# sk4161/EgoScaler

Hardware: AMD Instinct MI355X
Metric: clips/sec/GPU (8-frame 224^2, 16-token text) fwd+bwd (higher is better)
Workload: dtype bf16

## Files before the change

### egoscaler_amd/csrc/elementwise.hip

```cpp
#include "common.h"
#include <math.h>

template <typename T>
__global__ __launch_bounds__(256) void layernorm_fwd_kernel(const T* x, const T* add, const T* w, const T* b, T* sum_out, T* y,
                                                            int rows, int cols, float eps) {
    const int row = blockIdx.x * 4 + (threadIdx.x >> 6), lane = threadIdx.x & 63;
    if (row >= rows) return;
    const T* xr = x + (long long)row * cols;
    const T* ar = add ? add + (long long)row * cols : nullptr;
    float s = 0.f;
    for (int c = lane; c < cols; c += 64) {
        float v = Cvt<T>::ld(xr + c);
        if (ar) v += Cvt<T>::ld(ar + c);
        s += v;
    }
    const float mean = wave_sum(s) / cols;
    float q = 0.f;
    for (int c = lane; c < cols; c += 64) {
        float v = Cvt<T>::ld(xr + c);
        if (ar) v += Cvt<T>::ld(ar + c);
        if (sizeof(T) == 2) v = bf2f(f2bf(v));
        const float dlt = v - mean;
        q += dlt * dlt;
    }
// ... 861 lines not shown
#pragma unroll
        for (int j = 0; j < 4; ++j) {
            float pi = p4[j], mi = m4[j], vi = v4[j];
            adamw_elem(pi, mi, vi, g4[j], lr, b1, b2, eps, wd, bc1, bc2_sqrt, gscale);
            p4[j] = pi; m4[j] = mi; v4[j] = vi;
        }
        reinterpret_cast<f32x4*>(p)[i] = p4; reinterpret_cast<f32x4*>(m)[i] = m4; reinterpret_cast<f32x4*>(v)[i] = v4;
        if (p_model) {
            T o[4];
#pragma unroll
            for (int j = 0; j < 4; ++j) Cvt<T>::st(o + j, p4[j]);
            typedef T tx4 __attribute__((ext_vector_type(4)));
            reinterpret_cast<tx4*>(p_model)[i] = tx4{o[0], o[1], o[2], o[3]};
        }
    }
}

template <typename G>
static int adamw_launch(float* master, void* model_copy, const G* grad, float* m, float* v, int64_t n, float lr, float beta1, float beta2, float eps,
                        float weight_decay, int step, float grad_scale, int copy_dtype, hipStream_t stream) {
    if (!master || !grad || !m || !v) return EGOMI_E_BADARG;
    if (n <= 0 || step <= 0) return EGOMI_E_SHAPE;
    if (model_copy && copy_dtype != EGOMI_F32 && copy_dtype != EGOMI_BF16) return EGOMI_E_BADARG;
    const float bc1 = 1.0f - powf(beta1, (float)step), bc2s = sqrtf(1.0f - powf(beta2, (float)step));
    const long long n4 = n / 4, rest = n - 4 * n4;
    const bool vec = n4 > 0 && (((uintptr_t)master | (uintptr_t)m | (uintptr_t)v) & 15) == 0 && ((uintptr_t)grad & (4 * sizeof(G) - 1)) == 0 &&
                     (!model_copy || (copy_dtype == EGOMI_BF16 && ((uintptr_t)model_copy & 7) == 0));
    if (vec) {
        EGOMI_LAUNCH((adamw_vec4_kernel<bf16_t, G>), dim3(ew_grid(n4)), dim3(256), 0, stream, master, (bf16_t*)model_copy, grad, m, v,
                           n4, lr, beta1, beta2, eps, weight_decay, bc1, bc2s, grad_scale);
        if (rest == 0) return egomi_launch_status();
        master += 4 * n4; grad += 4 * n4; m += 4 * n4; v += 4 * n4; n = rest;
        if (model_copy) model_copy = (bf16_t*)model_copy + 4 * n4;
    }
    if (!model_copy || copy_dtype == EGOMI_F32)
        EGOMI_LAUNCH((adamw_kernel<float, G>), dim3(ew_grid(n)), dim3(256), 0, stream, master, (float*)model_copy, grad, m, v,
                           (long long)n, lr, beta1, beta2, eps, weight_decay, bc1, bc2s, grad_scale);
    else
        EGOMI_LAUNCH((adamw_kernel<bf16_t, G>), dim3(ew_grid(n)), dim3(256), 0, stream, master, (bf16_t*)model_copy, grad, m, v,
                           (long long)n, lr, beta1, beta2, eps, weight_decay, bc1, bc2s, grad_scale);
    return egomi_launch_status();
}

extern "C" int egomi_adamw(float* master, void* model_copy, const float* grad, float* m, float* v, int64_t n, float lr, float beta1,
                           float beta2, float eps, float weight_decay, int step, float grad_scale, int copy_dtype, egomi_stream_t stream) {
    return adamw_launch<float>(master, model_copy, grad, m, v, n, lr, beta1, beta2, eps, weight_decay, step, grad_scale, copy_dtype, (hipStream_t)stream);
}
extern "C" int egomi_adamw_g16(float* master, void* model_copy, const void* grad_bf16, float* m, float* v, int64_t n, float lr, float beta1,
                               float beta2, float eps, float weight_decay, int step, float grad_scale, int copy_dtype, egomi_stream_t stream) {
    return adamw_launch<bf16_t>(master, model_copy, (const bf16_t*)grad_bf16, m, v, n, lr, beta1, beta2, eps, weight_decay, step, grad_scale, copy_dtype,
                                (hipStream_t)stream);
}

template <typename T>
__global__ __launch_bounds__(256) void transpose_kernel(const T* in, int R, int C, long long ldi, T* out, long long ldo) {
    __shared__ T tile[32][33];
    const int c0 = blockIdx.x * 32, r0 = blockIdx.y * 32;
    const int tx = threadIdx.x & 31, ty = threadIdx.x >> 5;
    for (int i = ty; i < 32; i += 8) {
        const int r = r0 + i, c = c0 + tx;
        tile[i][tx] = (r < R && c < C) ? in[(long long)r * ldi + c] : (T)0;
    }
    __syncthreads();
    for (int i = ty; i < 32; i += 8) {
        const int c = c0 + i, r = r0 + tx;
        if (c < C && r < ldo) out[(long long)c * ldo + r] = tile[tx][i];
    }
}

__global__ __launch_bounds__(256) void transpose_bf16_vec_kernel(const bf16_t* in, int R, int C, long long ldi, bf16_t* out, long long ldo) {
    __shared__ __attribute__((aligned(16))) bf16_t tile[64][72];
    const int c0 = blockIdx.x * 64, r0 = blockIdx.y * 64;
    const int t = threadIdx.x;
#pragma unroll
    for (int i = 0; i < 2; ++i) {
        const int r = (t >> 3) + 32 * i, cc = (t & 7) * 8;
        u32x4 v = {0u, 0u, 0u, 0u};
        if (r0 + r < R && c0 + cc < C) v = *reinterpret_cast<const u32x4*>(in + (long long)(r0 + r) * ldi + c0 + cc);
        *reinterpret_cast<u32x4*>(&tile[r][cc]) = v;
    }
    __syncthreads();
#pragma unroll
    for (int i = 0; i < 2; ++i) {
        const int oc = (t >> 3) + 32 * i, rc = (t & 7) * 8;
        if (c0 + oc >= C || r0 + rc >= ldo) continue;
        u32x4 v;
#pragma unroll
        for (int j = 0; j < 4; ++j) v[j] = (uint32_t)tile[rc + 2 * j][oc] | ((uint32_t)tile[rc + 2 * j + 1][oc] << 16);
        *reinterpret_cast<u32x4*>(out + (long long)(c0 + oc) * ldo + r0 + rc) = v;
    }
}

extern "C" int egomi_transpose(const void* in, int R, int C, int64_t ldi, void* out, int64_t ldo, int dtype, egomi_stream_t stream) {
    if (!in || !out) return EGOMI_E_BADARG;
    if (R <= 0 || C <= 0 || ldi < C || ldo < R) return EGOMI_E_SHAPE;
    if (dtype == EGOMI_BF16 && C % 8 == 0 && ldi % 8 == 0 && ldo % 8 == 0 && ((uintptr_t)in % 16) == 0 && ((uintptr_t)out % 16) == 0) {
        dim3 g((C + 63) / 64, (unsigned)((ldo + 63) / 64));
        EGOMI_LAUNCH(transpose_bf16_vec_kernel, g, dim3(256), 0, (hipStream_t)stream, (const bf16_t*)in, R, C, (long long)ldi, (bf16_t*)out, (long long)ldo);
        return egomi_launch_status();
    }
    dim3 grid((C + 31) / 32, (unsigned)((ldo + 31) / 32));
    EGOMI_DISPATCH_DTYPE(dtype, EGOMI_LAUNCH(transpose_kernel<T>, grid, dim3(256), 0, (hipStream_t)stream, (const T*)in, R, C, ldi, (T*)out, ldo));
    return egomi_launch_status();
}

template <typename TI, typename TO>
// ... 148 lines not shown
```

### egoscaler_amd/engine.py

```python
import os
import types
from typing import Dict

import torch

from . import lora, ops
from .config import EgoDims


class Workspace:

    def __init__(self, device):
        self.device = device
        self.bufs: Dict[str, torch.Tensor] = {}

    def get(self, name, shape, dtype, zero=False):
        t = self.bufs.get(name)
        shape = tuple(int(s) for s in shape)
        if t is None or t.shape != shape or t.dtype != dtype:
            t = self.bufs[name] = torch.empty(shape, dtype=dtype, device=self.device)
        if zero:
            t.zero_()
        return t

    def bytes(self):
        return sum(t.numel() * t.element_size() for t in self.bufs.values())


class Engine:
    def __init__(self, dims: EgoDims, params: Dict[str, torch.Tensor], device, dtype):
        self.dims, self.w, self.device, self.dtype = dims, params, device, dtype
        self.ws = Workspace(device)
        self.w8 = None
        self.w4 = None
        self.prepared = False
        self.prepare_epoch = 0
        self.lm_wT, self.lm_wT_stale, self.lm_wT_ver = None, True, None
        self.param_ref = {}
        self.grad_fresh = set()
        self._xt_last = {}
        self.main_grad: Dict[str, torch.Tensor] = {}
        self.layer_flat: Dict[int, torch.Tensor] = {}
        self.trainable: Dict[str, bool] = {}
        self.ctx = None
        self.grad_sync = None
        self.pb_drop_override = None
        self.reduced_grad = {}
        self.layer_offs = {}
        self._direct, self._direct_done = None, set()
        self.layer_final_hook = None
        self.param_events = {}
        self.use_fused_attention = True
        self.use_fused_swiglu = os.environ.get("EGOMI_NO_FUSED_SWIGLU", "0") != "1"
        self.use_tail_fuse = os.environ.get("EGOMI_NO_TAIL_FUSE", "0") != "1"
        self.use_tn = os.environ.get("EGOMI_GEMM_TN", "1") != "0"
        self.use_top_rows = os.environ.get("EGOMI_TOP_ROWS", "1") != "0"
        self.top_rows_taken = 0
        self._top_key = None
        self.pb_trainer = None
        self.defer_splice_check = False
        self.pending_splice = None
        self._splice_host = {}
        self.pb_train_mode = False
        self.prepared_bn_stale = False
        self.fold_stale = False
        self.lora = None
        self.lora_version = 0
        self._lora_ws = None

    @staticmethod
    def param_group_of(name):
        if name.startswith("model.layers."):
            return int(name.split(".")[2])
        if name == "model.embed_tokens.weight":
            return "embed"
        if name in ("model.norm.weight", "lm_head.weight"):
            return "post"
        return "pre"

    def wait_params(self, key):
        ev = self.param_events.pop(key, None)
        if ev is not None:
            torch.cuda.current_stream().wait_event(ev)

    def wait_param_updates(self):
        for key in list(self.param_events):
            self.wait_params(key)

    def _notify(self, name):
        if self.grad_sync is not None and name in self.trainable and name in self.main_grad:
            self.grad_sync.ready(name, self.main_grad[name])

    def _notify_layer(self, l):
        one_rank = self.grad_sync is None or getattr(self.grad_sync, "local", False)
        hook = self.layer_final_hook if one_rank else None
        if self.grad_sync is None or l not in self.layer_flat:
            if hook is not None:
                hook(l)
            return
        if self._direct is not None:
            wire, views = self._direct
            for n, v in views.items():
                if n not in self._direct_done:
                    if n in self.grad_fresh:
                        self.main_grad[n].zero_()
                        self.grad_fresh.discard(n)
                    ops.cast(self.main_grad[n].view(-1), wire.dtype, out=v.view(-1))
                self.reduced_grad[n] = v
            self._direct, self._direct_done = None, set()
            self.grad_sync.ready_resident(f"layer{l}", wire)
            if hook is not None:
                hook(l)
            return
        self.grad_sync.ready_flat(f"layer{l}", self.layer_flat[l])
        if hook is not None:
            hook(l)
    def _begin_direct(self, l):
        self._direct, self._direct_done = None, set()
        gs = self.grad_sync
        if gs is None or not getattr(gs, "resident", False) or not self.use_tn or self.dtype != torch.bfloat16:
            return
        names = [n for n in self.layer_param_names(l) if n in self.trainable]
        if not names:
            return
        if l not in self.layer_flat:
            self._alloc_layer_grads(l)
        if any(self.w[n].dim() == 2 and n not in self.grad_fresh for n in names):
            return
        wire = gs.resident_wire(f"layer{l}", self.layer_flat[l].numel(), self.device)
        if wire is None:
            return
# ... 78 lines not shown
            if t.data_ptr() != end or t.untyped_storage().data_ptr() != t0.untyped_storage().data_ptr():
                return None
            end += t.numel() * t.element_size()
        return torch.as_strided(t0, (sum(t.shape[0] for t in ts), t0.shape[1]), (t0.shape[1], 1))

    def stack_gate_up(self, gate, up):
        if not self.gu_il:
            return torch.cat([gate, up], 0)
        Fd = gate.shape[0]
        return torch.stack([gate.view(Fd // 32, 32, -1), up.view(Fd // 32, 32, -1)], 1).reshape(2 * Fd, -1).contiguous()

    def after_weights_update(self):
        self.lm_wT_stale = True
        if self.lora is not None and any(lora.is_adapter(n) for n in self.trainable):
            self.lora_version += 1
        if not self.prepared:
            return
        if self.pb_trainable:
            self.fold_stale = True
        for nm, wt in self.wT.items():
            if nm in self.trainable:
                ops.transpose(self.w[nm], out=wt)

    def set_trainable(self, names):
        self.trainable = {n: True for n in names}

    def grad_buffer(self, name):
        g = self.main_grad.get(name)
        if g is None:
            if name.startswith("model.layers."):
                self._alloc_layer_grads(int(name.split(".")[2]))
                return self.main_grad[name]
            g = torch.zeros(self.w[name].shape, dtype=torch.float32, device=self.device)
            self.main_grad[name] = g
        return g

    def _alloc_layer_grads(self, l):
        names = [n for n in self.layer_param_names(l) if n in self.trainable]
        offs, total = [], 0
        for n in names:
            offs.append(total)
            total += (self.w[n].numel() + 63) // 64 * 64
        flat = torch.zeros(total, dtype=torch.float32, device=self.device)
        self.layer_flat[l] = flat
        self.layer_offs[l] = dict(zip(names, offs))
        for n, o in zip(names, offs):
            self.main_grad[n] = flat[o:o + self.w[n].numel()].view(self.w[n].shape)

    def zero_grad(self):
        self.wait_param_updates()
        for g in self.main_grad.values():
            g.zero_()
        self.grad_fresh.clear()

    def lazy_zero_ok(self, name):
        return self.w[name].dim() == 2 and (name.startswith("model.layers.") or name == "lm_head.weight" or name.startswith("model.point_proj."))

    def flush_fresh(self):
        for n in list(self.grad_fresh):
            self.main_grad[n].zero_()
        self.grad_fresh.clear()

    def _attention(self, qkv, B, S, H, hd, out, causal, key_mask, scale, keep_P):
        d = H * hd
        T = self.dtype
        q, k, v = qkv[:, :d], qkv[:, d:2 * d], qkv[:, 2 * d:]
        sc = self.ws.get("att_scores", (B * H, S, S), torch.float32)
        ops.gemm_raw(q, k, sc, S, S, hd, 3 * d, 3 * d, S, 0, 0, alpha=scale, batch=B * H, batch_inner=H,
                     strides=(S * 3 * d, hd, S * 3 * d, hd, H * S * S, S * S))
        Pm = torch.empty(B * H, S, S, dtype=T, device=self.device) if keep_P else self.ws.get("att_P", (B * H, S, S), T)
        ops.softmax(sc, B * H, H, S, S, Pm, causal=causal, key_mask=key_mask)
        ops.gemm_raw(Pm, v, out, S, hd, S, S, 3 * d, d, 0, 1, batch=B * H, batch_inner=H,
                     strides=(H * S * S, S * S, S * 3 * d, hd, S * d, hd))
        return Pm

    def _attention_bwd(self, qkv, Pm, d_out, dqkv, B, S, H, hd, scale):
        d = H * hd
        q, k, v = qkv[:, :d], qkv[:, d:2 * d], qkv[:, 2 * d:]
        dq, dk, dv = dqkv[:, :d], dqkv[:, d:2 * d], dqkv[:, 2 * d:]
        dP = self.ws.get("att_scores", (B * H, S, S), torch.float32)
        ops.gemm_raw(d_out, v, dP, S, S, hd, d, 3 * d, S, 0, 0, batch=B * H, batch_inner=H,
                     strides=(S * d, hd, S * 3 * d, hd, H * S * S, S * S))
        dS = self.ws.get("att_dS", (B * H, S, S), self.dtype)
        ops.softmax_bwd(Pm, dP, dS, B * H * S, S)
        st_ss = (H * S * S, S * S)
        ops.gemm_raw(dS, k, dq, S, hd, S, S, 3 * d, 3 * d, 0, 1, alpha=scale, batch=B * H, batch_inner=H,
                     strides=(*st_ss, S * 3 * d, hd, S * 3 * d, hd))
        ops.gemm_raw(dS, q, dk, S, hd, S, S, 3 * d, 3 * d, 1, 1, alpha=scale, batch=B * H, batch_inner=H,
                     strides=(*st_ss, S * 3 * d, hd, S * 3 * d, hd))
        ops.gemm_raw(Pm, d_out, dv, S, hd, S, S, d, 3 * d, 1, 1, batch=B * H, batch_inner=H,
                     strides=(*st_ss, S * d, hd, S * 3 * d, hd))

    @torch.no_grad()
    def pointnet(self, nb2d, BG, K):
        if not self.prepared:
            self.prepare()
        if self.fold_stale:
            self.fold_batchnorm()
        w, pb, T, ws, f = self.w, self.dims.pb, self.dtype, self.ws, self.folded
        pre = "model.point_backbone."
        h1 = ops.linear_smallk(nb2d, f["c1_w"], f["c1_b"], act=ops.ACT_RELU, out=ws.get("pn_h1", (BG * K, pb.pn_c1), T))
        h2 = ops.mm(h1, f["c2_w"], out=ws.get("pn_h2", (BG * K, pb.pn_c2), T), bias=w[pre + "encoder.first_conv.3.bias"])
        cat = ops.group_max(h2, BG, K, pb.pn_c2, concat=True, out=ws.get("pn_cat", (BG * K, 2 * pb.pn_c2), T))
        h3 = ops.mm(cat, f["c3_w"], out=ws.get("pn_h3", (BG * K, pb.pn_c3), T), bias=f["c3_b"], act=ops.ACT_RELU)
        h4 = ops.mm(h3, f["c4_w"], out=ws.get("pn_h4", (BG * K, pb.encoder_dims), T), bias=w[pre + "encoder.second_conv.3.bias"])
        return ops.group_max(h4, BG, K, pb.encoder_dims, out=ws.get("pn_tok", (BG, pb.encoder_dims), T))
# ... 480 lines not shown
            else:
                ops.swiglu_bwd(d_act, gu[:, :Fd], gu[:, Fd:], dgu[:, :Fd], dgu[:, Fd:])
        self._wgrad(p + "down_proj.weight", dx, lc["act"])
        names = [p + "gate_proj.weight", p + "up_proj.weight"]
        d_h2, t_h2 = self._stacked_dgrad(dgu, wguT, self.wgu_cat.get(l) if self.prepared else None, names, ws.get("d_h" + sfx, (Ml, d), T),
                                         pl.defer_b and "gu" not in la, **mm)
        if "gu" in la:
            self._lora_bwd(l, "gu", dgu, lc["h2"], d_h2, lT["gu"], il=lc["gu_il"])
        self._wgrad_stacked(names, dgu, lc["h2"])
        n2 = f"model.layers.{l}.post_attention_layernorm.weight"
        return ops.rmsnorm_bwd(d_h2, lc["x_mid"], w[n2], lc["rstd2"], dx_add=dx, dw=self.grad_buffer(n2) if n2 in self.trainable else None,
                               out=ws.get("dx_b" + sfx, (Ml, d), T), tail=t_h2)

    def _attn_half_bwd(self, l, d_mid, lc, pl, key_mask):
        w, lm, T, ws, lw, la = self.w, self.dims.lm, self.dtype, self.ws, pl.layers[l], pl.la
        d, H, hd, B, S, M = lm.hidden_size, lm.num_attention_heads, lm.head_dim, pl.B, pl.S, pl.M
        p, qkv, lT = f"model.layers.{l}.self_attn.", lc["qkv"], lc["lora_T"]
        d_ao = self._dgrad(d_mid, p + "o_proj.weight", ws.get("d_ao" + ("_rows_top" if lw.top else ""), (lw.rows, d), T), **lw.mm)
        if "o" in la:
            self._lora_bwd(l, "o", d_mid, lc["ao"], d_ao, lT["o"])
        self._wgrad(p + "o_proj.weight", d_mid, lc["ao"])
        if lw.top:
            d_ao, d_mid = self._top_window(pl, self._top_buffers(B, S, pl.R)[2:], (d_ao, d_mid), scatter=True)
        dqkv = ws.get("dqkv", (M, 3 * d), T)
        if lc["lse"] is not None:
            ops.attn_bwd(qkv, lc["ao"], lc["lse"], d_ao, dqkv, ws.get("att_delta", (B, H, S), torch.float32), B, S, H, hd, hd ** -0.5,
                         causal=True, key_mask=key_mask, rope=(self.cos, self.sin), q_rows=pl.R if lw.top else 0)
        else:
            self._attention_bwd(qkv, lc["P"], d_ao, dqkv, B, S, H, hd, hd ** -0.5)
            ops.rope_(dqkv, self.cos, self.sin, M, S, 0, 2 * H, hd, 3 * d, inverse=True)
        names = [p + f"{nm}_proj.weight" for nm in "qkv"]
        stack = self.wqkv.get(l) if self.prepared and self.use_tn and T == torch.bfloat16 else None
        d_h, t_h = self._stacked_dgrad(dqkv, self.wqkvT.get(l) if self.prepared else None, stack, names, ws.get("d_h", (M, d), T),
                                       pl.defer_b and "qkv" not in la)
        if "qkv" in la:
            self._lora_bwd(l, "qkv", dqkv, lc["h"], d_h, lT["qkv"])
        self._wgrad_stacked(names, dqkv, lc["h"])
        n1 = f"model.layers.{l}.input_layernorm.weight"
        return ops.rmsnorm_bwd(d_h, lc["x_in"], w[n1], lc["rstd1"], dx_add=d_mid, dw=self.grad_buffer(n1) if n1 in self.trainable else None,
                               out=ws.get("dx_a", (M, d), T), tail=t_h)

    def _layer_bwd(self, l, dx, pl, ctx):
        lc = ctx["layers"][l]
        self._begin_direct(l)
        dx = self._attn_half_bwd(l, self._mlp_bwd(l, dx, lc, pl), lc, pl, ctx["key_mask"])
        self._notify_layer(l)
        return dx

    def _points_bwd(self, dx, ctx):
        w, pb, T, ws, tr = self.w, self.dims.pb, self.dtype, self.ws, self.trainable
        B, S, Bc, Pn, d = ctx["B"], ctx["S"], ctx["n_clouds"], pb.point_token_len, dx.shape[1]
        emb_name = "model.embed_tokens.weight"
        d_feats = ws.get("d_pp_out", (Bc * Pn, d), T, zero=True) if ctx["has_points"] else None
        ops.embed_splice_bwd(dx.view(B, S, d), ctx["ids"], ctx["start_pos"], Pn, self.dims.lm.vocab_size,
                             self.grad_buffer(emb_name) if emb_name in tr else None, d_feats, cloud_idx=ctx["cloud_idx"])
        if d_feats is None:
            return
        acts, g = ctx["pp_acts"], d_feats
        for j in range(len(pb.projection_hidden_dim), -1, -1):
            Wn, bn = f"model.point_proj.{2 * j}.weight", f"model.point_proj.{2 * j}.bias"
            self._wgrad(Wn, g, acts[2 * j])
            self._bgrad(bn, g)
            if j > 0:
                if T == torch.bfloat16:
                    wt = ops.transpose(w[Wn], out=ws.get(f"pp_wT{j}", (w[Wn].shape[1], w[Wn].shape[0]), T))
                    g_in = ops.mm(g, wt, out=ws.get(f"d_pp_act{j}", (Bc * Pn, w[Wn].shape[1]), T))
                else:
                    g_in = ops.mm(g, w[Wn], out=ws.get(f"d_pp_act{j}", (Bc * Pn, w[Wn].shape[1]), T), b_layout=1)
                g = ops.gelu_bwd(g_in, acts[2 * j - 1], out=ws.get(f"d_pp_pre{j}", g_in.shape, T))
            elif ctx.get("pb_ctx") is not None:
                d_backbone = ops.mm(g, w[Wn], b_layout=1)
                self.pb_trainer.backward(d_backbone.view(Bc, Pn, pb.trans_dim), ctx["pb_ctx"])
                if self.grad_sync is not None:
                    for nm in tr:
                        if nm.startswith("model.point_backbone."):
                            self._notify(nm)

    def backward_hidden(self, d_hn):
        ctx, w, ws, pl = self.ctx, self.w, self.ws, self.ctx["plan"]
        nf = "model.norm.weight"
        dx = ops.rmsnorm_bwd(d_hn, ctx["x_last"], w[nf], ctx["rstd_f"], dw=self.grad_buffer(nf) if nf in self.trainable else None,
                             out=ws.get("dx_a" + pl.layers[-1].sfx, ctx["x_last"].shape, self.dtype),
                             window=(pl.S, pl.R) if pl.R else None)
        for l in reversed(range(len(pl.layers))):
            dx = self._layer_bwd(l, dx, pl, ctx)
        self._points_bwd(dx, ctx)
        if self.grad_sync is not None:
            self._notify("model.embed_tokens.weight")
            self._notify(nf)
            for j in range(len(self.dims.pb.projection_hidden_dim) + 1):
                self._notify(f"model.point_proj.{2 * j}.weight")
                self._notify(f"model.point_proj.{2 * j}.bias")
            self.grad_sync.flush()
        self.ctx = None

    def layer_param_names(self, l):
        p = f"model.layers.{l}."
        names = [p + f"self_attn.{n}_proj.weight" for n in "qkvo"] + [p + f"mlp.{n}_proj.weight" for n in ("gate", "up", "down")] + \
                [p + "input_layernorm.weight", p + "post_attention_layernorm.weight"]
        if self.lora is not None:
            names += [n for t in self.lora.targets for n in lora.adapter_names(l, t)]
        return names

    def backward_logits(self, d_logits, hn):
        W = self.w["lm_head.weight"]
        V, d = W.shape
# ... 21 lines not shown
```

### egoscaler_amd/ops.py

```python
import ctypes
import math

import torch

from . import _abi, _lib
from ._lib import c_p, c_i, c_d, c_f, c_sz, c_i64, call, query

F32, BF16 = _abi.EGOMI_F32, _abi.EGOMI_BF16


def dt(t: torch.dtype) -> int:
    if t == torch.float32:
        return F32
    if t == torch.bfloat16:
        return BF16
    raise TypeError(f"unsupported dtype {t}")


def P(t):
    if t is None:
        return c_p(None)
    if not t.is_cuda:
        raise _lib.EgomiError("egoscaler_amd ops need CUDA/HIP tensors (no CPU fallback)")
    return c_p(t.data_ptr())
# ... 433 lines not shown
    call("egomi_gelu_bwd", dy, x, out, x.numel(), dt(x.dtype), S())
    return out


def softmax(scores, Z, heads, Sq, Sk, out, causal=False, q_offset=0, key_mask=None):
    call("egomi_softmax_fwd", scores, Sk, key_mask, Z, heads, Sq, Sk, int(causal), q_offset, out, Sk, dt(out.dtype), S())
    return out


def softmax_bwd(Pm, dP, dS, rows, Sk):
    call("egomi_softmax_bwd", Pm, Sk, dP, Sk, dS, Sk, rows, Sk, dt(Pm.dtype), S())
    return dS


def splice_scan(ids, tok, Pn, n_clouds=None):
    B, Sl = ids.shape
    sp, err, cloud, scratch = (torch.empty(B, dtype=torch.int32, device=ids.device) for _ in range(4))
    call("egomi_splice_scan", ids, B, Sl, tok.point_patch, tok.point_start, tok.point_end, Pn, B if n_clouds is None else n_clouds, sp, err, cloud,
         scratch, S())
    return sp, err, cloud


def embed_splice(ids, W, feats, start_pos, Pn, out=None, cloud_idx=None):
    B, Sl = ids.shape
    V, d = W.shape
    out = torch.empty(B, Sl, d, dtype=W.dtype, device=W.device) if out is None else out
    call("egomi_embed_splice_fwd", ids, W, feats, start_pos, cloud_idx, B, Sl, d, Pn, V, out, dt(W.dtype), S())
    return out


def embed_splice_bwd(dout, ids, start_pos, Pn, V, dW=None, dfeats=None, cloud_idx=None):
    B, Sl, d = dout.shape
    call("egomi_embed_splice_bwd", dout, ids, start_pos, cloud_idx, B, Sl, d, Pn, V, dW, dfeats, dt(dout.dtype), S())


def cross_entropy(logits, targets, ignore_index, dlogits=None, grad_scale=1.0):
    R, V = logits.shape
    cnt = torch.zeros(1, dtype=torch.int32, device=logits.device)
    ls = torch.zeros(1, dtype=torch.float32, device=logits.device)
    rows = torch.empty(R, dtype=torch.float32, device=logits.device)
    call("egomi_ce_count", targets, R, ignore_index, cnt, S())
    call("egomi_ce_fwd_bwd", logits, _ld(logits), targets, R, V, ignore_index, cnt, ls, rows, dlogits, _ld(dlogits) if dlogits is not None else 0,
         grad_scale, dt(logits.dtype), S())
    return ls, cnt


def adamw(master, model_copy, grad, m, v, lr, beta1, beta2, eps, wd, step, grad_scale=1.0):
    if grad.dtype not in (torch.float32, torch.bfloat16) or not grad.is_contiguous() or grad.numel() != master.numel():
        raise _lib.EgomiError("adamw: the gradient must be a contiguous fp32 or bf16 tensor of the parameter's size")
    call("egomi_adamw" if grad.dtype == torch.float32 else "egomi_adamw_g16", master, model_copy, grad, m, v, master.numel(), lr, beta1, beta2, eps,
         wd, step, grad_scale, dt(model_copy.dtype) if model_copy is not None else F32, S())


def transpose(x, ldo=None, out=None):
    R, C = x.shape
    ldo = R if ldo is None else ldo
    out = torch.empty(C, ldo, dtype=x.dtype, device=x.device) if out is None else out
    call("egomi_transpose", x, R, C, _ld(x), out, ldo, dt(x.dtype), S())
    return out


def cast(x, dtype, out=None):
    out = torch.empty(x.shape, dtype=dtype, device=x.device) if out is None else out
    call("egomi_cast", x, dt(x.dtype), out, dt(dtype), x.numel(), S())
    return out


def rank_sum(chunks, out):
    W, c = chunks.shape
    call("egomi_rank_sum", chunks, dt(chunks.dtype), W, c, out, dt(out.dtype), S())
    return out


def add(a, b, out=None):
    out = torch.empty_like(a) if out is None else out
    call("egomi_add", a, b, out, a.numel(), dt(a.dtype), S())
    return out


def colsum_(x, out):
    R, C = x.shape
    call("egomi_colsum", x, R, C, _ld(x), out, dt(x.dtype), S())
    return out


def group_max(x, BG, M, C, concat=False, out=None):
    if out is None:
        out = torch.empty((BG * M, 2 * C) if concat else (BG, C), dtype=x.dtype, device=x.device)
    call("egomi_group_max", x, BG, M, C, out, int(concat), dt(x.dtype), S())
    return out


def linear_smallk(x, w, b, act=0, out=None):
    R, K = x.numel() // x.shape[-1], x.shape[-1]
    N = w.shape[0]
    out = torch.empty(R, N, dtype=w.dtype, device=w.device) if out is None else out
    call("egomi_linear_smallk", x, dt(x.dtype), w, b, out, R, N, K, act, dt(w.dtype), S())
    return out


AttnDesc = _abi.STRUCTS["egomi_attn_desc"]


def _attn_desc(qkv, B, Sq, H, hd, scale, causal, key_mask):
    d = AttnDesc()
    dm = H * hd
# ... 88 lines not shown
```

### egoscaler_amd/optim.py

```python
import torch

from . import ops


class EgoAdamW:
    def __init__(self, model, lr=2e-5, betas=(0.9, 0.999), eps=1e-8, weight_decay=0.01):
        self.model, self.lr, self.betas, self.eps, self.wd = model, lr, betas, eps, weight_decay
        self.t = 0
        self.state = {}
        for n, p in model.named_parameters():
            if p.requires_grad:
                master = p.data if p.dtype == torch.float32 else p.data.float()
                self.state[n] = {"p": p, "master": master, "m": torch.zeros_like(master), "v": torch.zeros_like(master)}

    def arm(self, grad_scale=1.0, lr=None):
        eng = self.model.engine
        self._armed = None
        eng.layer_final_hook = None
        if (eng.grad_sync is not None and not getattr(eng.grad_sync, "local", False)) or eng.device.type != "cuda" or not eng.any_layer_trainable:
            return False
        if any(nm in eng.trainable for nm in getattr(eng, "wT", {})):
            return False
        groups = {}
        for n in self.state:
            groups.setdefault(eng.param_group_of(n), []).append(n)
        self._armed = {"lr": self.lr if lr is None else lr, "grad_scale": grad_scale, "done": set(), "groups": groups}
        eng.layer_final_hook = self._early_layer
        return True

    def _early_layer(self, l):
        a, eng = self._armed, self.model.engine
        names = a["groups"].get(l)
        if not names or any(nm in eng.trainable for nm in eng.wT):
            return
        if getattr(self, "_side", None) is None:
            self._side = torch.cuda.Stream()
        self._side.wait_stream(torch.cuda.current_stream())
        with torch.cuda.stream(self._side):
            for n in names:
                self._update(n, self.state[n], eng, a["lr"], a["grad_scale"], t=self.t + 1)
            ev = torch.cuda.Event()
            ev.record(self._side)
            eng.param_events[l] = ev
        a["done"].add(l)

    def _update(self, n, st, eng, lr, grad_scale, t=None):
        g = eng.reduced_grad.get(n)
        if g is None:
            g = eng.main_grad.get(n)
        if g is None:
            return
        p = st["p"]
        copy = None if p.dtype == torch.float32 else p.data
        ops.adamw(st["master"], copy, g, st["m"], st["v"], lr, self.betas[0], self.betas[1], self.eps, self.wd, self.t if t is None else t, grad_scale)

    def step(self, grad_scale=1.0, lr=None, overlap=False):
        self.t += 1
        lr = self.lr if lr is None else lr
        eng = self.model.engine
        armed, self._armed = getattr(self, "_armed", None), None
        eng.layer_final_hook = None
        early = armed["done"] if armed is not None else set()
        if early and (armed["lr"] != lr or armed["grad_scale"] != grad_scale):
            raise RuntimeError("EgoAdamW.step: lr / grad_scale differ from the ones given to arm()")
        if not (overlap and eng.device.type == "cuda" and not any(nm in eng.trainable for nm in eng.wT)):
            eng.wait_param_updates()
            for n, st in self.state.items():
                if eng.param_group_of(n) not in early:
                    self._update(n, st, eng, lr, grad_scale)
            eng.after_weights_update()
            return
        groups = {}
        for n in self.state:
            groups.setdefault(eng.param_group_of(n), []).append(n)
        L = eng.dims.lm.num_hidden_layers
        order = ["pre", "embed"] + list(range(L)) + ["post"]
        cur = torch.cuda.current_stream()
        if getattr(self, "_side", None) is None:
            self._side = torch.cuda.Stream()
        self._side.wait_stream(cur)
        with torch.cuda.stream(self._side):
            for key in order:
                names = groups.get(key)
                if not names or key in early:
                    continue
                for n in names:
                    self._update(n, self.state[n], eng, lr, grad_scale)
                ev = torch.cuda.Event()
                ev.record(self._side)
                eng.param_events[key] = ev
        eng.after_weights_update()

    def zero_grad(self):
        self.model.engine.zero_grad()
        for st in self.state.values():
            st["p"].grad = None

    def state_dict(self):
        self.model.engine.wait_param_updates()
        return {"t": self.t, "state": {n: {k: st[k] for k in ("master", "m", "v")} for n, st in self.state.items()}}

    def state_dict_cpu(self):
        self.model.engine.wait_param_updates()
        return {"t": self.t, "state": {n: {k: st[k].detach().cpu() for k in ("master", "m", "v")} for n, st in self.state.items()}}

    def resync_masters(self):
        self.model.engine.wait_param_updates()
        for st in self.state.values():
            if st["p"].dtype != torch.float32:
                st["p"].data.copy_(st["master"])
        self.model.engine.after_weights_update()

    def load_state_dict(self, sd):
        self.model.engine.wait_param_updates()
        self.t = sd["t"]
        for n, s in sd["state"].items():
            for k in ("master", "m", "v"):
                self.state[n][k].copy_(s[k])


def linear_warmup_lr(base_lr, step, total_steps, warmup_steps=None):
    warm = int(total_steps / 5) if warmup_steps is None else int(warmup_steps)
    if step < warm:
        return base_lr * float(step) / float(max(1, warm))
    return base_lr * max(0.0, float(total_steps - step) / float(max(1, total_steps - warm)))
```

### egoscaler_amd/pointllm/model_arch.py

```python
import json
import os
import types
from dataclasses import dataclass
from typing import List, Optional, Tuple

import torch
import torch.nn as nn

from ..config import EgoDims, LlamaDims, PointBertDims, SpecialTokens
from ..engine import Engine
from .. import lora, ops, synth


class PointLLMConfig:
    model_type = "pointllm"

    def __init__(self, **kw):
        self.hidden_size = 4096
        self.intermediate_size = 11008
        self.num_hidden_layers = 32
        self.num_attention_heads = 32
        self.vocab_size = 32003
        self.rms_norm_eps = 1e-6
        self.rope_theta = 10000.0
# ... 275 lines not shown
        if hasattr(self.args, "lora_r"):
            self.args.lora_r = 0
        tr = [n for n in eng.trainable if not lora.is_adapter(n)]
        self.engine = None
        self._build_engine()
        self.engine.set_trainable(tr)
        return self

    def _build_engine(self):
        tensors = {k: v for k, v in self.named_parameters()}
        tensors.update({k: v for k, v in self.named_buffers()})
        dtype = self.model.embed_tokens.weight.dtype
        dev = self.model.embed_tokens.weight.device
        old = self.engine
        self.__dict__.pop("_decoders", None)
        self.__dict__.pop("_scorers", None)
        self.engine = Engine(self.dims, {k: v.data for k, v in tensors.items()}, dev, dtype)
        self.engine.param_ref = dict(self.named_parameters())
        self.engine.lora = self.lora_cfg
        if old is not None:
            self.engine.trainable = old.trainable
        pb = self.dims.pb
        cfg = self.point_backbone_config or {}
        cfg.update({"point_cloud_dim": pb.point_dims, "backbone_output_dim": pb.trans_dim,
                    "project_output_dim": self.dims.lm.hidden_size, "point_token_len": pb.point_token_len,
                    "mm_use_point_start_end": True, "projection_hidden_layer": len(pb.projection_hidden_dim),
                    "projection_hidden_dim": list(pb.projection_hidden_dim), "use_max_pool": False})
        self.point_backbone_config = cfg
        self.model.point_backbone_config = cfg
        self.model.load_point_backbone_checkpoint = self.load_point_backbone_checkpoint

    def get_model(self):
        return self.model

    def state_dict(self, *a, **k):
        if getattr(self, "engine", None) is not None:
            self.engine.wait_param_updates()
        return super().state_dict(*a, **k)

    def _apply(self, fn, *a, **k):
        if getattr(self, "engine", None) is not None:
            self.engine.wait_param_updates()
        r = super()._apply(fn, *a, **k)
        if getattr(self, "engine", None) is not None:
            self._build_engine()
        return r

    def load_state_dict(self, sd, strict=True, **kw):
        self.engine.wait_param_updates()
        r = super().load_state_dict(sd, strict=strict, **kw)
        self.engine.prepared = False
        self.engine.lm_wT_stale = True
        self.engine.lora_version += 1
        return r

    def load_pretrained_weights(self):
        files = sorted(f for f in os.listdir(self.model_name) if f.endswith(".safetensors"))
        sd = {}
        if files:
            from safetensors.torch import load_file
            for f in files:
                sd.update(load_file(os.path.join(self.model_name, f)))
        else:
            for f in sorted(f for f in os.listdir(self.model_name) if f.startswith("pytorch_model") and f.endswith(".bin")):
                sd.update(torch.load(os.path.join(self.model_name, f), map_location="cpu", weights_only=True))
        if sd:
            self.load_state_dict(sd, strict=False)

    def load_point_backbone_checkpoint(self, checkpoint_path=None):
        path = checkpoint_path if checkpoint_path is not None else getattr(self.config, "point_backbone_ckpt", None)
        if path is None:
            raise ValueError("no checkpoint path: pass one or set config.point_backbone_ckpt")
        ckpt = torch.load(path, map_location="cpu", weights_only=True)
        pre, dst = "module.point_encoder.", "model.point_backbone."
        src = {k[len(pre):]: v for k, v in ckpt["state_dict"].items() if k.startswith(pre)}
        own = {k[len(dst):]: v for k, v in super().state_dict().items() if k.startswith(dst)}
        self.engine.wait_param_updates()
        with torch.no_grad():
            for k, v in src.items():
                if k in own:
                    if own[k].shape != v.shape:
                        raise RuntimeError(f"size mismatch for {k}: copying a param with shape {tuple(v.shape)} from checkpoint, "
                                           f"the shape in current model is {tuple(own[k].shape)}.")
                    own[k].copy_(v)
        missing = [k for k in own if k not in src]
        unexpected = [k for k in src if k not in own]
        self.engine.prepared = False
        if not missing and not unexpected:
            print(f"PointBERT's weights are successfully loaded from {path}")
        else:
            print("missing_keys", missing, "unexpected_keys", unexpected)
        return types.SimpleNamespace(missing_keys=missing, unexpected_keys=unexpected)

    def save_pretrained(self, path):
        from safetensors.torch import save_file
        if isinstance(self.config, PointLLMConfig):
            self.config.save_pretrained(path)
        os.makedirs(path, exist_ok=True)
        save_file({k: v.detach().cpu().contiguous() for k, v in self.state_dict().items()}, os.path.join(path, "model.safetensors"))

    def _configure_trainable_parameters(self):
        unfreeze_pc = bool(getattr(self.args, "unfreeze_pc_encoder", False))
        unfreeze_llm = bool(getattr(self.args, "unfreeze_language_model", False))
        names = []
        for n, p in self.named_parameters():
            if n.startswith("model.point_backbone."):
# ... 13 lines not shown
        if new_num_tokens == old:
            return
        for name in ("model.embed_tokens.weight", "lm_head.weight"):
            mod, leaf = self, name
            parts = name.split(".")
            for q in parts[:-1]:
                mod = getattr(mod, q)
            w = getattr(mod, parts[-1])
            nw = torch.empty(new_num_tokens, w.shape[1], dtype=w.dtype, device=w.device)
            n = min(old, new_num_tokens)
            nw[:n] = w.data[:n]
            if new_num_tokens > old:
                nw[old:].normal_(0.0, 0.02)
            mod.register_parameter(parts[-1], nn.Parameter(nw, requires_grad=w.requires_grad))
        self.dims.lm.vocab_size = new_num_tokens
        if hasattr(self.config, "vocab_size"):
            self.config.vocab_size = new_num_tokens
        tr = self.engine.trainable
        self.engine = None
        self._build_engine()
        self.engine.trainable = tr
        self.engine.main_grad, self.engine.layer_flat = {}, {}

    def initialize_tokenizer_point_backbone_config_wo_embedding(self, tokenizer):
        cfg = self.point_backbone_config
        pp = getattr(self.config, "DEFAULT_POINT_PATCH_TOKEN", "<point_patch>")
        tokenizer.add_tokens([pp], special_tokens=True)
        cfg["default_point_patch_token"] = pp
        cfg["point_patch_token"] = tokenizer.convert_tokens_to_ids([pp])[0]
        ps = getattr(self.config, "DEFAULT_POINT_START_TOKEN", "<point_start>")
        pe = getattr(self.config, "DEFAULT_POINT_END_TOKEN", "<point_end>")
        tokenizer.add_tokens([ps, pe], special_tokens=True)
        cfg["default_point_start_token"], cfg["default_point_end_token"] = ps, pe
        cfg["point_start_token"] = tokenizer.convert_tokens_to_ids([ps])[0]
        cfg["point_end_token"] = tokenizer.convert_tokens_to_ids([pe])[0]
        self.set_point_token_ids(cfg["point_patch_token"], cfg["point_start_token"], cfg["point_end_token"])

    def set_point_token_ids(self, patch, start, end):
        t = self.dims.tok
        t.point_patch, t.point_start, t.point_end = int(patch), int(start), int(end)
        self.point_backbone_config.update(point_patch_token=int(patch), point_start_token=int(start), point_end_token=int(end))

    def _begin_backward(self, explicit=False):
        eng = self.engine
        eng._xt_last.clear()
        for n, p in self.named_parameters():
            if n in eng.trainable:
                g = eng.grad_buffer(n)
                fresh = (p.grad is None) if (p.dtype == torch.float32 and not explicit) else (not self.accumulate_grads)
                if fresh:
                    if eng.lazy_zero_ok(n):
                        eng.grad_fresh.add(n)
                    else:
                        g.zero_()

    def _publish_grads(self):
        eng = self.engine
        eng.flush_fresh()
        for n, p in self.named_parameters():
            if n in eng.trainable:
                g = eng.reduced_grad.get(n, eng.main_grad[n])
                p.main_grad = g
                if p.dtype == torch.float32:
                    p.grad = g

    def forward(self, input_ids=None, attention_mask=None, past_key_values=None, inputs_embeds=None, labels=None,
                use_cache=None, output_attentions=None, output_hidden_states=None, point_clouds=None, return_dict=None,
                fps_start=None):
        dev = self.engine.device
        input_ids = input_ids.to(dev)
        if fps_start is None and point_clouds is not None:
            n = point_clouds[0].shape[0] if isinstance(point_clouds, (list, tuple)) else point_clouds.shape[1]
            b = len(point_clouds) if isinstance(point_clouds, (list, tuple)) else point_clouds.shape[0]
            fps_start = torch.randint(0, n, (b,), dtype=torch.long)
        save = torch.is_grad_enabled() and self.training_graph
        logits = _LogitsFn.apply(self._anchor, self, input_ids, attention_mask, point_clouds, fps_start, save)
        out = CausalLMOutput(logits=logits)
        return out if (return_dict is None or return_dict) else (logits,)

    def loss_and_backward(self, input_ids, attention_mask, point_clouds, prompt_len, pad_token_id, fps_start=None,
                          backward=True, grad_scale=1.0):
        eng = self.engine
        dev = eng.device
        input_ids = input_ids.to(dev)
        B, S = input_ids.shape
        if fps_start is None and point_clouds is not None:
            fps_start = torch.randint(0, point_clouds.shape[1], (B,), dtype=torch.long)
        Lp = int(prompt_len)
        hn = eng.forward_hidden(input_ids, attention_mask, point_clouds, fps_start, save=backward, loss_from=Lp - 1 if backward else None)
        d = hn.shape[1]
        R = eng.ctx.get("top_rows", 0) if backward else 0
        if R:
            hs = hn.view(B, R, d)[:, :R - 1].reshape(-1, d)
        else:
            hs = hn.view(B, S, d)[:, Lp - 1:S - 1].reshape(-1, d)
        tg = input_ids[:, Lp:].reshape(-1).contiguous()
        lg = eng.logits(hs, padded=backward)
        ls, cnt = ops.cross_entropy(lg, tg, pad_token_id, dlogits=lg if backward else None, grad_scale=grad_scale)
        loss = ls / cnt.float()
        if backward:
            self._begin_backward(explicit=True)
            d_hs = eng.backward_logits(lg, hs)
            if R:
                eng.backward_hidden(eng.compact_loss_grad(d_hs))
            else:
                d_hn = eng.ws.get("d_hn_full", (B, S, d), eng.dtype, zero=True)
                d_hn[:, Lp - 1:S - 1] = d_hs.view(B, S - Lp, d)
# ... 216 lines not shown
```

### include/egomi.h

```cpp
#ifndef EGOMI_H
#define EGOMI_H
#include <stddef.h>
#include <stdint.h>

#ifdef __cplusplus
extern "C" {
#endif

#define EGOMI_OK 0
#define EGOMI_E_BADARG (-1)
#define EGOMI_E_SHAPE (-2)
#define EGOMI_E_LAUNCH (-3)
#define EGOMI_E_UNSUPPORTED (-4)

#define EGOMI_F32 0
#define EGOMI_BF16 1

typedef void* egomi_stream_t;

int egomi_version(void);
const char* egomi_strerror(int code);
const char* egomi_last_launch_error(void);

size_t egomi_unproject_workspace_bytes(int B, int T, int H, int W);
// ... 179 lines not shown
int egomi_rowscale_add(const void* resid, const void* branch, const float* scale, int64_t rows, int cols, int rows_per_sample, void* out,
                       int dtype, egomi_stream_t stream);

int egomi_layernorm_fwd(const void* x, const void* add, const void* w, const void* b, void* sum_out, void* y,
                        int rows, int cols, float eps, int dtype, egomi_stream_t stream);

int egomi_rmsnorm_fwd(const void* x, const void* w, void* y, float* rstd, int rows, int cols, float eps, int dtype,
                      egomi_stream_t stream);
int egomi_rmsnorm_bwd(const void* dy, const void* x, const void* w, const float* rstd, void* dx, const void* dx_add,
                      float* dw, int rows, int cols, int dtype, egomi_stream_t stream);
int egomi_rmsnorm_bwd_rows(const void* dy, const void* x, const void* w, const float* rstd, void* dx, const void* dx_add,
                           float* dw, int rows, int cols, int seq, int win, int dtype, egomi_stream_t stream);
int egomi_rmsnorm_fwd_tail(void* x, const void* w, void* y, float* rstd, int rows, int cols, float eps, int row0, const float* slabs, int slices,
                           const void* residual, int64_t ldr, int dtype, egomi_stream_t stream);
int egomi_rmsnorm_bwd_tail(void* dy, const void* x, const void* w, const float* rstd, void* dx, const void* dx_add, float* dw, int rows,
                           int cols, int row0, const float* slabs, int slices, int dtype, egomi_stream_t stream);

int egomi_rope(void* x, const float* cos_tab, const float* sin_tab, int64_t rows, int S, int pos_offset, int H, int hd,
               int64_t ld, int inverse, int dtype, egomi_stream_t stream);
int egomi_rope_qkv_tail(void* qkv, const float* cos_tab, const float* sin_tab, int64_t rows, int S, int pos_offset, int H, int hd, int64_t ld,
                        int row0, const float* slabs, int slices, int dtype, egomi_stream_t stream);

int egomi_swiglu_fwd(const void* gate, const void* up, void* out, int64_t rows, int cols, int64_t ld_in, int64_t ld_out,
                     int dtype, egomi_stream_t stream);
int egomi_swiglu_bwd(const void* dact, const void* gate, const void* up, void* dgate, void* dup, int64_t rows, int cols,
                     int64_t ld_in, int64_t ld_act, int64_t ld_out, int dtype, egomi_stream_t stream);
int egomi_swiglu_il_fwd(const void* gu, void* out, int64_t rows, int cols, int64_t ld_gu, int64_t ld_out, int dtype, egomi_stream_t stream);
int egomi_swiglu_il_bwd(const void* dact, const void* gu, void* dgu, int64_t rows, int cols, int64_t ld_gu, int64_t ld_act, int64_t ld_dgu,
                        int dtype, egomi_stream_t stream);

int egomi_gelu_fwd(const void* x, void* y, int64_t n, int dtype, egomi_stream_t stream);
int egomi_gelu_bwd(const void* dy, const void* x, void* dx, int64_t n, int dtype, egomi_stream_t stream);

int egomi_softmax_fwd(const float* scores, int64_t ld_s, const uint8_t* key_mask, int Z, int heads, int Sq, int Sk, int causal,
                      int q_offset, void* P, int64_t ld_p, int dtype, egomi_stream_t stream);
int egomi_softmax_bwd(const void* P, int64_t ld_p, const float* dP, int64_t ld_dp, void* dS, int64_t ld_ds, int64_t rows, int Sk,
                      int dtype, egomi_stream_t stream);

int egomi_splice_scan(const int64_t* ids, int B, int S, int64_t patch_id, int64_t start_id, int64_t end_id, int P, int n_clouds,
                      int32_t* start_pos, int32_t* err, int32_t* cloud_idx, int32_t* scratch, egomi_stream_t stream);
int egomi_embed_splice_fwd(const int64_t* ids, const void* W, const void* feats, const int32_t* start_pos, const int32_t* cloud_idx,
                           int B, int S, int d, int P, int V, void* out, int dtype, egomi_stream_t stream);
int egomi_embed_splice_bwd(const void* dout, const int64_t* ids, const int32_t* start_pos, const int32_t* cloud_idx, int B, int S, int d,
                           int P, int V, float* dW, void* dfeats, int dtype, egomi_stream_t stream);

int egomi_ce_count(const int64_t* targets, int64_t n, int64_t ignore, int32_t* count, egomi_stream_t stream);
int egomi_ce_fwd_bwd(const void* logits, int64_t ld, const int64_t* targets, int R, int V, int64_t ignore, const int32_t* count,
                     float* loss_sum, float* row_loss, void* dlogits, int64_t ldd, float grad_scale, int dtype, egomi_stream_t stream);

int egomi_adamw(float* master, void* model_copy, const float* grad, float* m, float* v, int64_t n, float lr, float beta1,
                float beta2, float eps, float weight_decay, int step, float grad_scale, int copy_dtype, egomi_stream_t stream);
int egomi_adamw_g16(float* master, void* model_copy, const void* grad_bf16, float* m, float* v, int64_t n, float lr, float beta1,
                    float beta2, float eps, float weight_decay, int step, float grad_scale, int copy_dtype, egomi_stream_t stream);

int egomi_transpose(const void* in, int R, int C, int64_t ldi, void* out, int64_t ldo, int dtype, egomi_stream_t stream);
int egomi_cast(const void* in, int in_dtype, void* out, int out_dtype, int64_t n, egomi_stream_t stream);
int egomi_add(const void* a, const void* b, void* out, int64_t n, int dtype, egomi_stream_t stream);
int egomi_rank_sum(const void* in, int in_dtype, int W, int64_t c, void* out, int out_dtype, egomi_stream_t stream);
int egomi_colsum(const void* x, int64_t R, int C, int64_t ld, float* out, int dtype, egomi_stream_t stream);

int egomi_group_max(const void* x, int BG, int M, int C, void* out, int concat, int dtype, egomi_stream_t stream);
int egomi_linear_smallk(const void* x, int x_dtype, const void* w, const void* b, void* y, int64_t R, int N, int K, int act,
                        int dtype, egomi_stream_t stream);

#ifdef __cplusplus
}
#endif
#endif
```

Baseline: 68.37.

## Add row-sparse AdamW and masked grad zeroing for the embedding table

Adds a row-wise AdamW kernel for the token embedding. It skips reading and writing the m/v state for rows whose gradient is all zero and whose optimizer state has never been touched. It records which rows were updated so the next step zeroes only those gradient rows instead of the whole buffer. With 16 text tokens per clip, most of the large vocab embedding rows are untouched, which should cut optimizer and zeroing memory traffic. The cost is extra bookkeeping (live/touched masks) and subtle state invariants across steps and state-dict loads.

```diff
diff --git a/egoscaler_amd/csrc/elementwise.hip b/egoscaler_amd/csrc/elementwise.hip
--- a/egoscaler_amd/csrc/elementwise.hip
+++ b/egoscaler_amd/csrc/elementwise.hip
@@ -937,6 +937,128 @@
                                 (hipStream_t)stream);
 }
 
+template <typename G, int NS>
+__global__ __launch_bounds__(256) void adamw_rows_kernel(float* p, bf16_t* p_model, const G* g, float* m, float* v, long long rows, int c4,
+                                                         uint8_t* live, uint8_t* touched, float lr, float b1, float b2, float eps, float wd,
+                                                         float bc1, float bc2_sqrt, float gscale) {
+    typedef float f32x4 __attribute__((ext_vector_type(4)));
+    for (long long r = blockIdx.x; r < rows; r += gridDim.x) {
+        const long long base = r * c4;
+        const int was_live = live[r];
+        f32x4 g4[NS], p4[NS];
+        uint32_t nz = 0;
+#pragma unroll
+        for (int s = 0; s < NS; ++s) {
+            const int c = s * 256 + (int)threadIdx.x;
+            if (c < c4) {
+                if constexpr (sizeof(G) == 4) {
+                    g4[s] = __builtin_nontemporal_load(reinterpret_cast<const f32x4*>(g) + base + c);
+#pragma unroll
+                    for (int j = 0; j < 4; ++j) nz |= __float_as_uint(g4[s][j]) & 0x7FFFFFFFu;
+                } else {
+                    const u32x2 w = __builtin_nontemporal_load(reinterpret_cast<const u32x2*>(g) + base + c);
+                    g4[s][0] = __uint_as_float(w[0] << 16); g4[s][1] = __uint_as_float(w[0] & 0xFFFF0000u);
+                    g4[s][2] = __uint_as_float(w[1] << 16); g4[s][3] = __uint_as_float(w[1] & 0xFFFF0000u);
+                    nz |= (w[0] | w[1]) & 0x7FFF7FFFu;
+                }
+                p4[s] = reinterpret_cast<const f32x4*>(p)[base + c];
+            }
+        }
+        const bool full = (__syncthreads_or(nz != 0) != 0) || was_live != 0;
+#pragma unroll
+        for (int s = 0; s < NS; ++s) {
+            const int c = s * 256 + (int)threadIdx.x;
+            if (c < c4) {
+                f32x4 q4 = p4[s];
+                if (full) {
+                    f32x4 m4 = reinterpret_cast<f32x4*>(m)[base + c], v4 = reinterpret_cast<f32x4*>(v)[base + c];
+#pragma unroll
+                    for (int j = 0; j < 4; ++j) {
+                        float pi = q4[j], mi = m4[j], vi = v4[j];
+                        adamw_elem(pi, mi, vi, g4[s][j], lr, b1, b2, eps, wd, bc1, bc2_sqrt, gscale);
+                        q4[j] = pi; m4[j] = mi; v4[j] = vi;
+                    }
+                    reinterpret_cast<f32x4*>(m)[base + c] = m4; reinterpret_cast<f32x4*>(v)[base + c] = v4;
+                } else {
+#pragma unroll
+                    for (int j = 0; j < 4; ++j) {
+                        float pi = q4[j], mi = 0.0f, vi = 0.0f;
+                        adamw_elem(pi, mi, vi, g4[s][j], lr, b1, b2, eps, wd, bc1, bc2_sqrt, gscale);
+                        q4[j] = pi;
+                    }
+                }
+                reinterpret_cast<f32x4*>(p)[base + c] = q4;
+                if (p_model) {
+                    bf16_t o[4];
+#pragma unroll
+                    for (int j = 0; j < 4; ++j) Cvt<bf16_t>::st(o + j, q4[j]);
+                    typedef bf16_t bx4 __attribute__((ext_vector_type(4)));
+                    reinterpret_cast<bx4*>(p_model)[base + c] = bx4{o[0], o[1], o[2], o[3]};
+                }
+            }
+        }
+        if (threadIdx.x == 0) {
+            if (full) live[r] = 1;
+            touched[r] = full ? 1 : 0;
+        }
+    }
+}
+
+template <typename G>
+static int adamw_rows_launch(float* master, void* model_copy, const G* grad, float* m, float* v, int64_t rows, int64_t cols, uint8_t* live,
+                             uint8_t* touched, float lr, float beta1, float beta2, float eps, float weight_decay, int step, float grad_scale,
+                             int copy_dtype, hipStream_t stream) {
+    if (!master || !grad || !m || !v || !live || !touched) return EGOMI_E_BADARG;
+    if (rows <= 0 || cols <= 0 || step <= 0) return EGOMI_E_SHAPE;
+    if (model_copy && copy_dtype != EGOMI_F32 && copy_dtype != EGOMI_BF16) return EGOMI_E_BADARG;
+    if (!(eps > 0.0f) || !std::isfinite(grad_scale) || !std::isfinite(beta1) || !std::isfinite(beta2)) return EGOMI_E_UNSUPPORTED;
+    if (cols % 4 != 0 || cols > 4 * 256 * 8) return EGOMI_E_UNSUPPORTED;
+    if ((((uintptr_t)master | (uintptr_t)m | (uintptr_t)v) & 15) != 0 || ((uintptr_t)grad & (4 * sizeof(G) - 1)) != 0 ||
+        (model_copy && (copy_dtype != EGOMI_BF16 || ((uintptr_t)model_copy & 7) != 0)))
+        return EGOMI_E_UNSUPPORTED;
+    const float bc1 = 1.0f - powf(beta1, (float)step), bc2s = sqrtf(1.0f - powf(beta2, (float)step));
+    const int c4 = (int)(cols / 4);
+    const dim3 grid((unsigned)(rows < 2048 ? rows : 2048));
+#define EGOMI_ADAMW_ROWS(NS)                                                                                                              \
+    EGOMI_LAUNCH((adamw_rows_kernel<G, NS>), grid, dim3(256), 0, stream, master, (bf16_t*)model_copy, grad, m, v, (long long)rows, c4, live, \
+                 touched, lr, beta1, beta2, eps, weight_decay, bc1, bc2s, grad_scale)
+    if (c4 <= 256) EGOMI_ADAMW_ROWS(1);
+    else if (c4 <= 512) EGOMI_ADAMW_ROWS(2);
+    else if (c4 <= 1024) EGOMI_ADAMW_ROWS(4);
+    else EGOMI_ADAMW_ROWS(8);
+#undef EGOMI_ADAMW_ROWS
+    return egomi_launch_status();
+}
+
+extern "C" int egomi_adamw_rows(float* master, void* model_copy, const float* grad, float* m, float* v, int64_t rows, int64_t cols, uint8_t* live,
+                                uint8_t* touched, float lr, float beta1, float beta2, float eps, float weight_decay, int step, float grad_scale,
+                                int copy_dtype, egomi_stream_t stream) {
+    return adamw_rows_launch<float>(master, model_copy, grad, m, v, rows, cols, live, touched, lr, beta1, beta2, eps, weight_decay, step, grad_scale,
+                                    copy_dtype, (hipStream_t)stream);
+}
+extern "C" int egomi_adamw_rows_g16(float* master, void* model_copy, const void* grad_bf16, float* m, float* v, int64_t rows, int64_t cols,
+                                    uint8_t* live, uint8_t* touched, float lr, float beta1, float beta2, float eps, float weight_decay, int step,
+                                    float grad_scale, int copy_dtype, egomi_stream_t stream) {
+    return adamw_rows_launch<bf16_t>(master, model_copy, (const bf16_t*)grad_bf16, m, v, rows, cols, live, touched, lr, beta1, beta2, eps,
+                                     weight_decay, step, grad_scale, copy_dtype, (hipStream_t)stream);
+}
+
+__global__ __launch_bounds__(256) void zero_rows_kernel(float* buf, long long rows, int c4, const uint8_t* mask) {
+    typedef float f32x4 __attribute__((ext_vector_type(4)));
+    const long long r = (long long)blockIdx.x * 4 + (threadIdx.x >> 6);
+    if (r >= rows || mask[r] == 0) return;
+    f32x4* row = reinterpret_cast<f32x4*>(buf) + r * c4;
+    for (int c = threadIdx.x & 63; c < c4; c += 64) row[c] = f32x4{0.0f, 0.0f, 0.0f, 0.0f};
+}
+
+extern "C" int egomi_zero_rows(float* buf, int64_t rows, int64_t cols, const uint8_t* mask, egomi_stream_t stream) {
+    if (!buf || !mask) return EGOMI_E_BADARG;
+    if (rows <= 0 || cols <= 0 || cols / 4 > 0x7FFFFFFF || (rows + 3) / 4 > 0x7FFFFFFF) return EGOMI_E_SHAPE;
+    if (cols % 4 != 0 || ((uintptr_t)buf & 15) != 0) return EGOMI_E_UNSUPPORTED;
+    EGOMI_LAUNCH(zero_rows_kernel, dim3((unsigned)((rows + 3) / 4)), dim3(256), 0, (hipStream_t)stream, buf, (long long)rows, (int)(cols / 4), mask);
+    return egomi_launch_status();
+}
+
 template <typename T>
 __global__ __launch_bounds__(256) void transpose_kernel(const T* in, int R, int C, long long ldi, T* out, long long ldo) {
     __shared__ T tile[32][33];
diff --git a/egoscaler_amd/engine.py b/egoscaler_amd/engine.py
--- a/egoscaler_amd/engine.py
+++ b/egoscaler_amd/engine.py
@@ -42,6 +42,7 @@
         self.main_grad: Dict[str, torch.Tensor] = {}
         self.layer_flat: Dict[int, torch.Tensor] = {}
         self.trainable: Dict[str, bool] = {}
+        self.grad_rows = {}
         self.ctx = None
         self.grad_sync = None
         self.pb_drop_override = None
@@ -77,6 +78,18 @@
         if name in ("model.norm.weight", "lm_head.weight"):
             return "post"
         return "pre"
+
+    @staticmethod
+    def row_sparse_grad(name):
+        return name == "model.embed_tokens.weight"
+
+    def clear_grad(self, name, g):
+        tok = self.grad_rows.pop(name, None)
+        if tok is not None and tok[0] is g:
+            self.wait_params(self.param_group_of(name))
+            ops.zero_rows(g, tok[1])
+        else:
+            g.zero_()
 
     def wait_params(self, key):
         ev = self.param_events.pop(key, None)
@@ -261,6 +274,7 @@
         for g in self.main_grad.values():
             g.zero_()
         self.grad_fresh.clear()
+        self.grad_rows.clear()
 
     def lazy_zero_ok(self, name):
         return self.w[name].dim() == 2 and (name.startswith("model.layers.") or name == "lm_head.weight" or name.startswith("model.point_proj."))
@@ -847,6 +861,7 @@
         B, S, Bc, Pn, d = ctx["B"], ctx["S"], ctx["n_clouds"], pb.point_token_len, dx.shape[1]
         emb_name = "model.embed_tokens.weight"
         d_feats = ws.get("d_pp_out", (Bc * Pn, d), T, zero=True) if ctx["has_points"] else None
+        self.grad_rows.pop(emb_name, None)
         ops.embed_splice_bwd(dx.view(B, S, d), ctx["ids"], ctx["start_pos"], Pn, self.dims.lm.vocab_size,
                              self.grad_buffer(emb_name) if emb_name in tr else None, d_feats, cloud_idx=ctx["cloud_idx"])
         if d_feats is None:
diff --git a/egoscaler_amd/ops.py b/egoscaler_amd/ops.py
--- a/egoscaler_amd/ops.py
+++ b/egoscaler_amd/ops.py
@@ -509,6 +509,28 @@
          wd, step, grad_scale, dt(model_copy.dtype) if model_copy is not None else F32, S())
 
 
+def adamw_rows(master, model_copy, grad, m, v, live, touched, lr, beta1, beta2, eps, wd, step, grad_scale=1.0):
+    rows, cols = master.shape
+    if grad.dtype not in (torch.float32, torch.bfloat16) or not grad.is_contiguous() or grad.shape != master.shape:
+        raise _lib.EgomiError("adamw_rows: the gradient must be a contiguous fp32 or bf16 tensor of the parameter's shape")
+    if live.dtype != torch.uint8 or touched.dtype != torch.uint8 or live.numel() != rows or touched.numel() != rows:
+        raise _lib.EgomiError("adamw_rows: live and touched are uint8 [rows]")
+    rc = query("egomi_adamw_rows" if grad.dtype == torch.float32 else "egomi_adamw_rows_g16", master, model_copy, grad, m, v, rows, cols, live,
+               touched, lr, beta1, beta2, eps, wd, step, grad_scale, dt(model_copy.dtype) if model_copy is not None else F32, S())
+    if rc == _abi.EGOMI_E_UNSUPPORTED:
+        adamw(master, model_copy, grad, m, v, lr, beta1, beta2, eps, wd, step, grad_scale)
+        return False
+    _lib.check(rc, "egomi_adamw_rows")
+    return True
+
+
+def zero_rows(buf, mask):
+    rows, cols = buf.shape
+    if buf.dtype != torch.float32 or not buf.is_contiguous() or mask.dtype != torch.uint8 or mask.numel() != rows:
+        raise _lib.EgomiError("zero_rows: a contiguous fp32 [rows, cols] buffer and a uint8 [rows] mask")
+    call("egomi_zero_rows", buf, rows, cols, mask, S())
+
+
 def transpose(x, ldo=None, out=None):
     R, C = x.shape
     ldo = R if ldo is None else ldo
diff --git a/egoscaler_amd/optim.py b/egoscaler_amd/optim.py
--- a/egoscaler_amd/optim.py
+++ b/egoscaler_amd/optim.py
@@ -1,3 +1,5 @@
+import os
+
 import torch
 
 from . import ops
@@ -12,6 +14,8 @@
             if p.requires_grad:
                 master = p.data if p.dtype == torch.float32 else p.data.float()
                 self.state[n] = {"p": p, "master": master, "m": torch.zeros_like(master), "v": torch.zeros_like(master)}
+        self.use_rows = os.environ.get("EGOMI_ADAMW_ROWS", "1") != "0"
+        self._rows = {}
 
     def arm(self, grad_scale=1.0, lr=None):
         eng = self.model.engine
@@ -52,7 +56,20 @@
             return
         p = st["p"]
         copy = None if p.dtype == torch.float32 else p.data
-        ops.adamw(st["master"], copy, g, st["m"], st["v"], lr, self.betas[0], self.betas[1], self.eps, self.wd, self.t if t is None else t, grad_scale)
+        t = self.t if t is None else t
+        if self.use_rows and eng.row_sparse_grad(n) and st["master"].dim() == 2 and g.is_contiguous():
+            rs = self._rows.get(n)
+            if rs is None:
+                bits = (st["m"].view(torch.int32) | st["v"].view(torch.int32)) != 0
+                rs = self._rows[n] = {"live": bits.any(dim=1).to(torch.uint8), "touched": torch.empty(bits.shape[0], dtype=torch.uint8, device=bits.device)}
+            took = ops.adamw_rows(st["master"], copy, g, st["m"], st["v"], rs["live"], rs["touched"], lr, self.betas[0], self.betas[1], self.eps, self.wd,
+                                  t, grad_scale)
+            if not took:
+                rs["live"].fill_(1)
+            elif g is eng.main_grad.get(n) and (eng.grad_sync is None or getattr(eng.grad_sync, "local", False)):
+                eng.grad_rows[n] = (g, rs["touched"])
+            return
+        ops.adamw(st["master"], copy, g, st["m"], st["v"], lr, self.betas[0], self.betas[1], self.eps, self.wd, t, grad_scale)
 
     def step(self, grad_scale=1.0, lr=None, overlap=False):
         self.t += 1
@@ -117,6 +134,8 @@
         for n, s in sd["state"].items():
             for k in ("master", "m", "v"):
                 self.state[n][k].copy_(s[k])
+        self._rows.clear()
+        self.model.engine.grad_rows.clear()
 
 
 def linear_warmup_lr(base_lr, step, total_steps, warmup_steps=None):
diff --git a/egoscaler_amd/pointllm/model_arch.py b/egoscaler_amd/pointllm/model_arch.py
--- a/egoscaler_amd/pointllm/model_arch.py
+++ b/egoscaler_amd/pointllm/model_arch.py
@@ -351,6 +351,7 @@
         self.engine.prepared = False
         self.engine.lm_wT_stale = True
         self.engine.lora_version += 1
+        self.engine.grad_rows.clear()
         return r
 
     def load_pretrained_weights(self):
@@ -470,7 +471,9 @@
                     if eng.lazy_zero_ok(n):
                         eng.grad_fresh.add(n)
                     else:
-                        g.zero_()
+                        eng.clear_grad(n, g)
+                else:
+                    eng.grad_rows.pop(n, None)
 
     def _publish_grads(self):
         eng = self.engine
diff --git a/include/egomi.h b/include/egomi.h
--- a/include/egomi.h
+++ b/include/egomi.h
@@ -255,6 +255,13 @@
                 float beta2, float eps, float weight_decay, int step, float grad_scale, int copy_dtype, egomi_stream_t stream);
 int egomi_adamw_g16(float* master, void* model_copy, const void* grad_bf16, float* m, float* v, int64_t n, float lr, float beta1,
                     float beta2, float eps, float weight_decay, int step, float grad_scale, int copy_dtype, egomi_stream_t stream);
+int egomi_adamw_rows(float* master, void* model_copy, const float* grad, float* m, float* v, int64_t rows, int64_t cols, uint8_t* live,
+                     uint8_t* touched, float lr, float beta1, float beta2, float eps, float weight_decay, int step, float grad_scale,
+                     int copy_dtype, egomi_stream_t stream);
+int egomi_adamw_rows_g16(float* master, void* model_copy, const void* grad_bf16, float* m, float* v, int64_t rows, int64_t cols,
+                         uint8_t* live, uint8_t* touched, float lr, float beta1, float beta2, float eps, float weight_decay, int step,
+                         float grad_scale, int copy_dtype, egomi_stream_t stream);
+int egomi_zero_rows(float* buf, int64_t rows, int64_t cols, const uint8_t* mask, egomi_stream_t stream);
 
 int egomi_transpose(const void* in, int R, int C, int64_t ldi, void* out, int64_t ldo, int dtype, egomi_stream_t stream);
 int egomi_cast(const void* in, int in_dtype, void* out, int out_dtype, int64_t n, egomi_stream_t stream);
```

After: 68.70 (median of 6 runs). No clear change (+0.5%).
